# cc-ai/climategan

Measured on AMD Instinct MI355X. Metric: 640x640 images/sec (G+D step): per-domain sample slots per second of the joint Masker+Painter training step (update_G + update_D), global batch 32 per domain, higher is better.
Workload: dtype bf16

## Files before the change

climategan_amd/csrc/conv_gemm.h:

```cpp
#pragma once
#include "cgan_common.h"

struct ConvGemmArgs {
  const uint16_t* x;
  const u32x4* w;
  const float* bias;
  const uint16_t* res;
  const uint16_t* res2;
  uint16_t* y;
  int n, h_in, w_in, cin_s;
  int cout, cout_s, ctiles, ksteps;
  int kh, kw, stride, pad, dil, pad_mode;
  int h_out, w_out, npix;
  int act, has_res, res_ups;
  float slope;
  float* stats;
};

struct ConvGemmCls {
  int koff;
  int kh, kw;
  int offy, offx;
};
struct ConvGemmExtArgs {
  ConvGemmArgs a;
  int cls_s;
  int ksplit;
  int ks_per;
  float* ws;
  int pair;
  ConvGemmCls cls[4];
};
bool conv_gemm_ext_shape_ok(const ConvGemmArgs& a);
int conv_gemm_splitk_plan(const ConvGemmArgs& a);
size_t conv_gemm_splitk_workspace_bytes(const ConvGemmArgs& a, int ksplit);
int conv_gemm_splitk_launch(const ConvGemmArgs& a, int ksplit, float* ws, int dtype, hipStream_t s);
int conv_gemm_cls_launch(const ConvGemmArgs& a, int cls_s, const ConvGemmCls* cls, int dtype, hipStream_t s);
int conv_gemm_pair_launch(const ConvGemmArgs& a, int dtype, hipStream_t s);

bool conv_gemm_applicable(const CganConvDesc* d);
int conv_gemm_launch(const ConvGemmArgs& a, int dtype, hipStream_t s);
bool conv_gemm_res2_ok(const ConvGemmArgs& a, int dtype);
int conv_gemm_stats_chunk_pixels(const ConvGemmArgs& a, int dtype);
bool conv_gemm_big_ok(const ConvGemmArgs& a);
bool conv1x1_allc_ok(const ConvGemmArgs& a);
int conv1x1_allc_launch(const ConvGemmArgs& a, int dtype, hipStream_t s);
int conv_gemm_big_launch(const ConvGemmArgs& a, int dtype, hipStream_t s);
bool conv_gemm_big_pair_ok(const ConvGemmArgs& a, int dtype);
int conv_gemm_big_pair_launch(const ConvGemmArgs& a, int dtype, hipStream_t s);
bool conv1x1_xres_ok(const ConvGemmArgs& a);
int conv1x1_xres_launch(const ConvGemmArgs& a, int dtype, hipStream_t s);

#ifdef __HIPCC__
typedef float f32x2 __attribute__((ext_vector_type(2)));

__device__ __forceinline__ float row16_sum(float v) {
  v += __builtin_bit_cast(float, __builtin_amdgcn_update_dpp(0, __builtin_bit_cast(int, v), 0x128, 0xf, 0xf, false));
  v += __builtin_bit_cast(float, __builtin_amdgcn_update_dpp(0, __builtin_bit_cast(int, v), 0x124, 0xf, 0xf, false));
  v += __builtin_bit_cast(float, __builtin_amdgcn_update_dpp(0, __builtin_bit_cast(int, v), 0x122, 0xf, 0xf, false));
  v += __builtin_bit_cast(float, __builtin_amdgcn_update_dpp(0, __builtin_bit_cast(int, v), 0x121, 0xf, 0xf, false));
  return v;
}

template <typename T, int WC, int WP>
__device__ __forceinline__ void conv_gemm_stats_epilogue(f32x4 (&acc)[WC][WP], const ConvGemmArgs& p, int cout_base,
                                                         int chunk, int j, int g) {
  if (p.bias) {
#pragma unroll
    for (int c = 0; c < WC; ++c) {
      const int chb = cout_base + c * 16 + 4 * g;
      const f32x4 b = chb < p.cout_s ? *reinterpret_cast<const f32x4*>(p.bias + chb) : (f32x4){0.f, 0.f, 0.f, 0.f};
#pragma unroll
      for (int t = 0; t < WP; ++t) acc[c][t] += b;
    }
  }
  constexpr float inv_cnt = 1.f / (float)(WP * 16);
#pragma unroll
  for (int c = 0; c < WC; ++c) {
    f32x2 vr[WP][2];
#pragma unroll
    for (int t = 0; t < WP; ++t) {
#pragma unroll
      for (int hh = 0; hh < 2; ++hh) {
        float r0, r1;
        unpack2<T>(pack2<T>(acc[c][t][2 * hh], acc[c][t][2 * hh + 1]), r0, r1);
        vr[t][hh] = (f32x2){r0, r1};
      }
    }
    f32x2 s0[2] = {vr[0][0], vr[0][1]};
#pragma unroll
    for (int t = 1; t < WP; ++t) {
      s0[0] += vr[t][0];
      s0[1] += vr[t][1];
    }
    float sm[4], sq[4];
#pragma unroll
    for (int r = 0; r < 4; ++r) sm[r] = row16_sum(s0[r >> 1][r & 1]) * inv_cnt;
    const f32x2 m2[2] = {(f32x2){sm[0], sm[1]}, (f32x2){sm[2], sm[3]}};
    f32x2 s1[2];
#pragma unroll
    for (int hh = 0; hh < 2; ++hh) {
      const f32x2 dv = vr[0][hh] - m2[hh];
      s1[hh] = dv * dv;
    }
// ... 141 lines not shown
```

climategan_amd/csrc/conv_gemm.hip:

```cpp
#include "conv_gemm.h"
#include <type_traits>

namespace {

__device__ __attribute__((aligned(16))) unsigned int g_gemm_zeros[4];

constexpr int NSTAGE = 3;
CGAN_KNOB(int, g_gemm_ws, 0);

__device__ __forceinline__ int reflect_i(int i, int n) {
  if (i < 0) i = -i;
  if (i >= n) i = 2 * n - 2 - i;
  return i;
}

template <typename T, int WAVES_C, int WC, int WP, bool REFLECT, int NS = NSTAGE, bool RES2 = false>
__global__ __launch_bounds__(256, 2) void conv_gemm_kernel(ConvGemmArgs p, int npb, int ncb) {
  constexpr int WAVES_P = 4 / WAVES_C;
  constexpr int CT_BLK = WAVES_C * WC;
  constexpr int PT_BLK = WAVES_P * WP;
  constexpr int STAGE_BYTES = (CT_BLK + PT_BLK) * 1024;
  constexpr int W_PER_WAVE = CT_BLK / 4;
  constexpr int P_PER_WAVE = PT_BLK / 4;
  constexpr int DMA_PER_WAVE = W_PER_WAVE + P_PER_WAVE;
  static_assert(CT_BLK % 4 == 0 && PT_BLK % 4 == 0, "tiles must split evenly over the 4 waves");
  extern __shared__ __attribute__((aligned(1024))) unsigned char smem[];

  const int lane = threadIdx.x & 63;
  const int wave = __builtin_amdgcn_readfirstlane(threadIdx.x >> 6);
  const int j = lane & 15;
  const int g = lane >> 4;
  const int wc = wave % WAVES_C, wp = wave / WAVES_C;

  const int xcd = blockIdx.x & 7, slot = blockIdx.x >> 3;
  const int cblk = slot % ncb;
  const int pblk = xcd * ((npb + 7) >> 3) + slot / ncb;
  if (pblk >= npb) return;

  int pbase[P_PER_WAVE], py0[P_PER_WAVE], px0[P_PER_WAVE];
#pragma unroll
  for (int m = 0; m < P_PER_WAVE; ++m) {
    int pix = (pblk * PT_BLK + wave + 4 * m) * 16 + j;
    bool v = pix < p.npix;
    int pc = v ? pix : 0;
    int ox = pc % p.w_out;
    int r = pc / p.w_out;
    int oy = r % p.h_out;
    int nn = r / p.h_out;
    pbase[m] = nn * p.h_in * p.w_in * p.cin_s + g * 8;
    py0[m] = v ? oy * p.stride - p.pad : -(1 << 28);
    px0[m] = ox * p.stride - p.pad;
  }
  const int ccn = p.cin_s >> 5;
  const long zero_off = reinterpret_cast<const unsigned char*>(g_gemm_zeros) - reinterpret_cast<const unsigned char*>(p.x);

  int i_ky = 0, i_kx = 0, i_cc = 0, i_buf = 0;
  auto issue_piece = [&](int piece) {
    unsigned char* buf = smem + i_buf * STAGE_BYTES;
    if (piece < W_PER_WAVE) {
      const int i = wave + 4 * piece;
      const int ct = min(cblk * CT_BLK + i, p.ctiles - 1);
      const u32x4* src = p.w + ((size_t)ct * p.ksteps + (i_ky * p.kw + i_kx) * ccn + i_cc) * 64 + lane;
      __builtin_amdgcn_global_load_lds((const __attribute__((address_space(1))) void*)src,
                                       (__attribute__((address_space(3))) void*)(buf + i * 1024), 16, 0, 0);
    } else {
      const int m = piece - W_PER_WAVE;
      const int i = wave + 4 * m;
      int iy = py0[m] + i_ky * p.dil, ix = px0[m] + i_kx * p.dil;
      bool ok;
      if (REFLECT) {
        ok = py0[m] > -(1 << 27);
        iy = reflect_i(ok ? iy : 0, p.h_in);
        ix = reflect_i(ix, p.w_in);
      } else {
        ok = (unsigned)iy < (unsigned)p.h_in && (unsigned)ix < (unsigned)p.w_in;
      }
      const long off = ok ? (long)(pbase[m] + (iy * p.w_in + ix) * p.cin_s + i_cc * 32) * 2 : zero_off;
      const unsigned char* src = reinterpret_cast<const unsigned char*>(p.x) + off;
      __builtin_amdgcn_global_load_lds((const __attribute__((address_space(1))) void*)src,
                                       (__attribute__((address_space(3))) void*)(buf + (CT_BLK + i) * 1024), 16, 0, 0);
    }
  };
  auto issue_advance = [&]() {
    const int kx1 = i_kx + 1;
    const bool wx = kx1 == p.kw;
    i_kx = wx ? 0 : kx1;
    const int ky1 = i_ky + (wx ? 1 : 0);
    const bool wy = ky1 == p.kh;
    i_ky = wy ? 0 : ky1;
    const int cc1 = i_cc + (wy ? 1 : 0);
    i_cc = cc1 == ccn ? 0 : cc1;
    i_buf = (i_buf + 1 == NS) ? 0 : i_buf + 1;
  };
  auto issue = [&]() {
#pragma unroll
    for (int q = 0; q < DMA_PER_WAVE; ++q) issue_piece(q);
    issue_advance();
  };

  f32x4 acc[WC][WP];
#pragma unroll
  for (int c = 0; c < WC; ++c)
#pragma unroll
    for (int t = 0; t < WP; ++t) acc[c][t] = (f32x4){0.f, 0.f, 0.f, 0.f};

  issue();
  if (NS > 2) issue();
  int r_buf = 0;
  for (int ks = 0; ks < p.ksteps; ++ks) {
    asm volatile("s_waitcnt vmcnt(%0) lgkmcnt(0)" ::"n"((NS - 2) * DMA_PER_WAVE) : "memory");
    __builtin_amdgcn_s_barrier();
    const unsigned char* buf = smem + r_buf * STAGE_BYTES;
    u32x4 a[WC], b[WP];
#pragma unroll
    for (int t = 0; t < WP; ++t)
      b[t] = *reinterpret_cast<const u32x4*>(buf + (CT_BLK + wp * WP + t) * 1024 + lane * 16);
#pragma unroll
    for (int c = 0; c < WC; ++c) a[c] = *reinterpret_cast<const u32x4*>(buf + (wc * WC + c) * 1024 + lane * 16);
    constexpr int NM = WC * WP;
    constexpr int GAP = NM / (DMA_PER_WAVE + 1);
    __builtin_amdgcn_sched_barrier(0);
#pragma unroll
    for (int i = 0; i < NM; ++i) {
      const int c = i / WP, t = i % WP;
      acc[c][t] = mfma16(as_vec8<T>(a[c]), as_vec8<T>(b[t]), acc[c][t]);
      if ((i + 1) % GAP == 0 && (i + 1) / GAP <= DMA_PER_WAVE) {
        issue_piece((i + 1) / GAP - 1);
        __builtin_amdgcn_sched_barrier(0);
      }
    }
    issue_advance();
    r_buf = (r_buf + 1 == NS) ? 0 : r_buf + 1;
  }

  constexpr int ROWB = WC * 64 + 16;
  constexpr int PP = (4 * 4 * 16 * ROWB <= NS * STAGE_BYTES && WP % 4 == 0) ? 4
                     : (4 * 2 * 16 * ROWB <= NS * STAGE_BYTES ? 2 : 1);
  static_assert(4 * PP * 16 * ROWB <= NS * STAGE_BYTES, "epilogue staging does not fit");
  static_assert(WP % PP == 0, "WP must be a multiple of PP");
  asm volatile("s_waitcnt vmcnt(0) lgkmcnt(0)" ::: "memory");
  __builtin_amdgcn_s_barrier();
  unsigned char* stg = smem + wave * (PP * 16 * ROWB);
  const int cout_base = (cblk * CT_BLK + wc * WC) * 16;
  const float* bias_ep = p.bias;
  if (p.stats && (pblk * PT_BLK + wp * WP) * 16 < p.npix) {
    conv_gemm_stats_epilogue<T, WC, WP>(acc, p, cout_base, pblk * WAVES_P + wp, j, g);
    if (p.bias) bias_ep = nullptr;
  }
  conv_gemm_staged_store<T, WC, WP, PP, RES2>(acc, p, stg, (pblk * PT_BLK + wp * WP) * 16, cout_base, bias_ep, lane, j, g);
}

template <typename T, int WC, int WP>
__global__ __launch_bounds__(512, 2) void conv_gemm_k64_kernel(ConvGemmArgs p, int npb, int ncb, int tiles_total) {
  constexpr int CT_BLK = 2 * WC, PT_BLK = 2 * WP;
  constexpr int W_BYTES = CT_BLK * 2048, STAGE_BYTES = (CT_BLK + PT_BLK) * 2048;
  constexpr int NS = 3;
  constexpr int W_PER = CT_BLK / 2, P_PER = PT_BLK / 2, PIECES = W_PER + P_PER;
  static_assert(PIECES <= 63, "vmcnt range");
  extern __shared__ __attribute__((aligned(1024))) unsigned char smem[];

  const int lane = threadIdx.x & 63;
  const int wave = __builtin_amdgcn_readfirstlane(threadIdx.x >> 6);
  const int xcd = blockIdx.x & 7, slot = blockIdx.x >> 3, nslot = gridDim.x >> 3;
  const int per = (tiles_total + 7) >> 3;
  const int t0 = xcd * per;
  const int t1 = min(t0 + per, tiles_total);
  const int my_n = (t1 - t0 > slot) ? (t1 - t0 - slot + nslot - 1) / nslot : 0;
  if (my_n <= 0) return;
  const int first = t0 + slot;
  const int cc2n = p.cin_s >> 6;
  const int n_st = p.kh * p.kw * cc2n;
  const int n_it = my_n * n_st;

  if (wave >= 4) {
    const int pw = wave - 4;
    const int half = pw & 1;
    const int ccn = p.cin_s >> 5;
    const long zero_off = reinterpret_cast<const unsigned char*>(g_gemm_zeros) - reinterpret_cast<const unsigned char*>(p.x);
    const int q = lane >> 3;
    const int kchunk = (lane & 7) ^ (4 * half + ((q >> 1) & 3));
    int poff[P_PER];
    unsigned vmask[P_PER];
    const u32x4* wtile[W_PER];
    auto set_tile = [&](int ti) {
      const int gt = first + ti * nslot;
      const int pblk = gt / ncb;
      const int cblk = gt - pblk * ncb;
#pragma unroll
      for (int m = 0; m < W_PER; ++m)
        wtile[m] = p.w + (size_t)min(cblk * CT_BLK + (pw >> 1) + 2 * m, p.ctiles - 1) * p.ksteps * 64 + half * 64 + lane;
#pragma unroll
      for (int m = 0; m < P_PER; ++m) {
        const int pix = (pblk * PT_BLK + (pw >> 1) + 2 * m) * 16 + 8 * half + q;
        const bool v = pix < p.npix;
        const int pc = v ? pix : 0;
        const int ox = pc % p.w_out;
        const int r = pc / p.w_out;
        const int oy = r % p.h_out;
        const int nn = r / p.h_out;
        const int py0 = oy * p.stride - p.pad, px0 = ox * p.stride - p.pad;
        poff[m] = ((nn * p.h_in * p.w_in + py0 * p.w_in + px0) * p.cin_s + kchunk * 8) * 2;
        unsigned mk = 0;
        for (int ky = 0; ky < p.kh; ++ky)
          for (int kx = 0; kx < p.kw; ++kx) {
            const bool ok = v && (unsigned)(py0 + ky * p.dil) < (unsigned)p.h_in && (unsigned)(px0 + kx * p.dil) < (unsigned)p.w_in;
            mk |= (ok ? 1u : 0u) << (ky * p.kw + kx);
          }
        vmask[m] = mk;
      }
    };
    int i_ky = 0, i_kx = 0, i_cc2 = 0, i_buf = 0, i_st = 0, i_tile = 0, issued = 0;
    auto issue_stage = [&]() {
      unsigned char* buf = smem + i_buf * STAGE_BYTES;
      const int tap = i_ky * p.kw + i_kx;
      const size_t w_ks = (size_t)(tap * ccn + 2 * i_cc2) * 64;
#pragma unroll
      for (int m = 0; m < W_PER; ++m)
        __builtin_amdgcn_global_load_lds((const __attribute__((address_space(1))) void*)(wtile[m] + w_ks),
                                         (__attribute__((address_space(3))) void*)(buf + (pw + 4 * m) * 1024), 16, 0, 0);
      const int tap_off = ((i_ky * p.w_in + i_kx) * p.dil * p.cin_s + i_cc2 * 64) * 2;
#pragma unroll
      for (int m = 0; m < P_PER; ++m) {
        const long off = ((vmask[m] >> tap) & 1u) ? (long)(poff[m] + tap_off) : zero_off;
        const unsigned char* src = reinterpret_cast<const unsigned char*>(p.x) + off;
        __builtin_amdgcn_global_load_lds((const __attribute__((address_space(1))) void*)src,
                                         (__attribute__((address_space(3))) void*)(buf + W_BYTES + (pw + 4 * m) * 1024), 16, 0, 0);
      }
      ++issued;
      i_buf = (i_buf + 1 == NS) ? 0 : i_buf + 1;
      if (++i_st == n_st) {
        i_st = 0; i_ky = 0; i_kx = 0; i_cc2 = 0;
        if (++i_tile < my_n) set_tile(i_tile);
      } else if (++i_kx == p.kw) {
        i_kx = 0;
        if (++i_ky == p.kh) {
          i_ky = 0;
          ++i_cc2;
        }
      }
    };
    set_tile(0);
    for (int s2 = 0; s2 < NS - 1; ++s2)
      if (issued < n_it) issue_stage();
    for (int j = 0; j < n_it; ++j) {
      if (issued - 1 - j >= NS - 2)
        asm volatile("s_waitcnt vmcnt(%0)" ::"n"((NS - 2) * PIECES) : "memory");
      else
        asm volatile("s_waitcnt vmcnt(0)" ::: "memory");
      __builtin_amdgcn_s_barrier();
      if (issued < n_it) issue_stage();
    }
    return;
  }

  const int wc = wave & 1, wp = wave >> 1;
  const int j16 = lane & 15, g = lane >> 4;
  f32x4 acc[WC][WP];
#pragma unroll
  for (int c = 0; c < WC; ++c)
#pragma unroll
    for (int t = 0; t < WP; ++t) acc[c][t] = (f32x4){0.f, 0.f, 0.f, 0.f};
  u32x4 a0[WC], b0[WP], a1[WC], b1[WP];
  int r_buf = 0;
  const int a_off = wc * WC * 2048 + lane * 16;
  int b_off[2];
  {
    const int q = j16 & 7, h = j16 >> 3;
#pragma unroll
    for (int c = 0; c < 2; ++c)
      b_off[c] = W_BYTES + wp * WP * 2048 + 1024 * h + 128 * q + 16 * ((4 * c + g) ^ (4 * h + ((q >> 1) & 3)));
  }
  auto fetch_one = [&](const unsigned char* buf, int c, int qi, u32x4* na, u32x4* nb) {
    if (qi < WP)
      nb[qi] = *reinterpret_cast<const u32x4*>(buf + b_off[c] + qi * 2048);
    else
      na[qi - WP] = *reinterpret_cast<const u32x4*>(buf + a_off + ((qi - WP) * 2 + c) * 1024);
  };
  auto step = [&](const u32x4* ca, const u32x4* cb, u32x4* na, u32x4* nb, int next_half) {
    __builtin_amdgcn_sched_barrier(0);
    if (next_half == 0) {
      asm volatile("s_waitcnt lgkmcnt(0)" ::: "memory");
      __builtin_amdgcn_s_barrier();
      r_buf = (r_buf + 1 == NS) ? 0 : r_buf + 1;
    }
    __builtin_amdgcn_sched_barrier(0);
// ... 34 lines not shown
            int ox = pix % p.w_out;
            int r = pix / p.w_out;
            int oy = r % p.h_out;
            int nn = r / p.h_out;
            rbase = (((size_t)nn * (p.h_out >> 1) + (oy >> 1)) * (p.w_out >> 1) + (ox >> 1)) * p.cout_s;
          } else {
            rbase = (size_t)pix * p.cout_s;
          }
        }
#pragma unroll
        for (int c = 0; c < WC; ++c) {
          const int ch = (cblk * CT_BLK + wc * WC + c) * 16 + 4 * g;
          rv[t][c] = make_uint2(0u, 0u);
          if (pix < p.npix && ch < p.cout_s) rv[t][c] = *reinterpret_cast<const uint2*>(p.res + rbase + ch);
        }
      }
      __builtin_amdgcn_sched_barrier(0);
      __builtin_amdgcn_s_waitcnt(0x0F70);
    }
#pragma unroll
    for (int t = 0; t < WP; ++t) {
      const int pix = (pblk * PT_BLK + wp * WP + t) * 16 + j16;
#pragma unroll
      for (int c = 0; c < WC; ++c) {
        const int ch = (cblk * CT_BLK + wc * WC + c) * 16 + 4 * g;
        float v[4] = {acc[c][t][0], acc[c][t][1], acc[c][t][2], acc[c][t][3]};
        acc[c][t] = (f32x4){0.f, 0.f, 0.f, 0.f};
        if (pix >= p.npix || ch >= p.cout_s) continue;
        if (p.bias) {
#pragma unroll
          for (int r = 0; r < 4; ++r) v[r] += p.bias[ch + r];
        }
        if (p.has_res) {
          float r0, r1;
          unpack2<T>(rv[t][c].x, r0, r1);
          v[0] = cgan_res_apply(v[0], r0, p.has_res); v[1] = cgan_res_apply(v[1], r1, p.has_res);
          unpack2<T>(rv[t][c].y, r0, r1);
          v[2] = cgan_res_apply(v[2], r0, p.has_res); v[3] = cgan_res_apply(v[3], r1, p.has_res);
        }
#pragma unroll
        for (int r = 0; r < 4; ++r) {
          v[r] = act_apply(v[r], p.act, p.slope);
          if (ch + r >= p.cout) v[r] = 0.f;
        }
        u32x2 o;
        o.x = pack2<T>(v[0], v[1]);
        o.y = pack2<T>(v[2], v[3]);
        CGAN_ST_STREAM(o, reinterpret_cast<u32x2*>(p.y + (size_t)pix * p.cout_s + ch));
      }
    }
  };

  for (int ti = 0; ti < my_n; ++ti) {
    first_read(ti > 0);
    for (int st = 0; st + 1 < n_st; ++st) {
      step(a0, b0, a1, b1, 1);
      step(a1, b1, a0, b0, 0);
    }
    step(a0, b0, a1, b1, 1);
    step(a1, b1, a0, b0, -1);
    epilogue(ti);
  }
}

template <typename T, int WC, int WP>
int launch_k64(const ConvGemmArgs& a, hipStream_t s) {
  constexpr int CT_BLK = 2 * WC, PT_BLK = 2 * WP;
  constexpr size_t smem = (size_t)3 * (CT_BLK + PT_BLK) * 2048;
  static bool attr_set = false;
  if (!attr_set) {
    hipError_t e = hipFuncSetAttribute(reinterpret_cast<const void*>(&conv_gemm_k64_kernel<T, WC, WP>),
                                       hipFuncAttributeMaxDynamicSharedMemorySize, 160 * 1024);
    if (e != hipSuccess) {
      cgan_set_error("conv_gemm_k64: hipFuncSetAttribute failed: %s", hipGetErrorString(e));
      return CGAN_ERR_HIP;
    }
    attr_set = true;
  }
  const int npb = ceil_div(ceil_div(a.npix, 16), PT_BLK);
  const int ncb = ceil_div(a.ctiles, CT_BLK);
  const int tiles = npb * ncb;
  const int per = ceil_div(tiles, 8);
  const int nslot = per < 32 ? per : 32;
  hipLaunchKernelGGL((conv_gemm_k64_kernel<T, WC, WP>), dim3(8 * nslot), dim3(512), smem, s, a, npb, ncb, tiles);
  return CGAN_OK;
}
bool k64_ok(const ConvGemmArgs& a) {
  return (a.cin_s & 63) == 0 && a.pad_mode != CGAN_PAD_REFLECT && a.kh * a.kw <= 32 &&
         (long)a.n * a.h_in * a.w_in * a.cin_s < (1L << 30) - (1L << 20);
}


template <typename T, int WAVES_C, int WC, int WP, bool REFLECT, int NS = NSTAGE, bool RES2 = false>
int launch_cfg2(const ConvGemmArgs& a, hipStream_t s) {
  constexpr int WAVES_P = 4 / WAVES_C;
  constexpr int CT_BLK = WAVES_C * WC, PT_BLK = WAVES_P * WP;
  constexpr size_t smem = (size_t)NS * (CT_BLK + PT_BLK) * 1024;
  static bool attr_set = false;
  if (!attr_set) {
    hipError_t e = hipFuncSetAttribute(reinterpret_cast<const void*>(&conv_gemm_kernel<T, WAVES_C, WC, WP, REFLECT, NS, RES2>),
                                       hipFuncAttributeMaxDynamicSharedMemorySize, 160 * 1024);
    if (e != hipSuccess) {
      cgan_set_error("conv_gemm: hipFuncSetAttribute failed: %s", hipGetErrorString(e));
      return CGAN_ERR_HIP;
    }
    attr_set = true;
  }
  const int npb = ceil_div(ceil_div(a.npix, 16), PT_BLK);
  const int ncb = ceil_div(a.ctiles, CT_BLK);
  const int grid = ceil_div(npb, 8) * 8 * ncb;
  hipLaunchKernelGGL((conv_gemm_kernel<T, WAVES_C, WC, WP, REFLECT, NS, RES2>), dim3(grid), dim3(256), smem, s, a, npb, ncb);
  return CGAN_OK;
}

template <typename T, int WAVES_C, int WC, int WP, int NS = NSTAGE>
int launch_cfg(const ConvGemmArgs& a, hipStream_t s) {
  return a.pad_mode == CGAN_PAD_REFLECT ? launch_cfg2<T, WAVES_C, WC, WP, true, NS>(a, s)
                                        : launch_cfg2<T, WAVES_C, WC, WP, false, NS>(a, s);
}

CGAN_KNOB(int, g_gemm_cfg, 0);

enum { KIND_PLAIN = 0, KIND_K64_256x128, KIND_K64_128x256, KIND_BIG, KIND_DIRECT, KIND_XRES };
struct Choice {
  int kind;
  int cfg;
};

Choice choose(const ConvGemmArgs& a, bool bf16) {
  const int ptiles = ceil_div(a.npix, 16);
  const bool no_big = g_gemm_ws == 9;
  const bool no_xres = g_gemm_ws == 9 || g_gemm_ws == 12;
  const int ws = (no_big || no_xres || g_gemm_ws == 13 || g_gemm_ws == 14) ? 0 : g_gemm_ws;
  switch (ws) {
    case 5: if (k64_ok(a)) return {KIND_K64_256x128, 0}; break;
    case 6: if (k64_ok(a)) return {KIND_K64_128x256, 0}; break;
    case 8: if (conv_gemm_big_ok(a)) return {KIND_BIG, 0}; break;
    case 10: if (conv1x1_allc_ok(a)) return {KIND_DIRECT, 0}; break;
    case 11: if (conv1x1_xres_ok(a)) return {KIND_XRES, 0}; break;
    default: break;
  }
  const bool automatic = ws == 0 && g_gemm_cfg == 0;
  (void)bf16;
  if (automatic && !no_big && conv1x1_allc_ok(a) && a.ctiles <= 4 && a.npix >= 16384) return {KIND_DIRECT, 0};
  if (automatic && !no_xres && conv1x1_xres_ok(a) && a.ctiles >= 16 && a.npix >= 16384) return {KIND_XRES, 0};
  const bool long_1x1 = a.kh * a.kw == 1 && g_gemm_ws != 13 &&
                        (g_gemm_ws == 14 ? (a.cin_s >= 2048 || (a.cin_s >= 512 && a.ctiles >= 128))
                                         : (a.cin_s >= 1024 || (a.cin_s >= 512 && a.ctiles >= 128)));
  if (automatic && !no_big && conv_gemm_big_ok(a) && a.npix >= 16384 &&
      ((a.cin_s * a.kh * a.kw >= 4096 && a.cin_s >= 512 && !(a.kh * a.kw >= 9 && a.cin_s >= 2048)) || long_1x1))
    return {KIND_BIG, 0};
  if (automatic && k64_ok(a) && a.kh * a.kw >= 9 && a.cin_s >= 512 && a.npix >= 16384) return {KIND_K64_256x128, 0};
  switch (g_gemm_cfg) {
    case 1: return {KIND_PLAIN, 1};
    case 2: if (a.ctiles <= 16) return {KIND_PLAIN, 2}; break;
    case 3: return {KIND_PLAIN, 3};
    case 4: return {KIND_PLAIN, 4};
    case 5: return {KIND_PLAIN, 5};
    default: break;
  }
  if (a.ctiles <= 4) return {KIND_PLAIN, 1};
  if (a.kh * a.kw == 1 && a.ksteps <= 16) return {KIND_PLAIN, 5};
  if (a.ctiles > 8 && a.ctiles <= 16 && ceil_div(ptiles, 8) >= 384) return {KIND_PLAIN, 2};
  if ((long)ceil_div(ptiles, 16) * ceil_div(a.ctiles, 8) >= 384) return {KIND_PLAIN, 3};
  return {KIND_PLAIN, 4};
}

template <typename T>
int launch(const ConvGemmArgs& a, hipStream_t s) {
  const Choice ch = choose(a, std::is_same<T, BF16>::value);
  switch (ch.kind) {
    case KIND_K64_256x128: return launch_k64<T, 8, 4>(a, s);
    case KIND_K64_128x256: return launch_k64<T, 4, 8>(a, s);
    case KIND_BIG: return conv_gemm_big_launch(a, T::id, s);
    case KIND_DIRECT: return conv1x1_allc_launch(a, T::id, s);
    case KIND_XRES: return conv1x1_xres_launch(a, T::id, s);
    default: break;
  }
  switch (ch.cfg) {
    case 1: return launch_cfg<T, 1, 4, 4>(a, s);
    case 2: return launch_cfg<T, 2, 8, 4>(a, s);
    case 3: return launch_cfg<T, 2, 4, 8>(a, s);
    case 5:
      if (a.has_res == 3) return launch_cfg2<T, 2, 4, 4, false, 2, true>(a, s);
      return launch_cfg<T, 2, 4, 4, 2>(a, s);
    default: return launch_cfg<T, 2, 4, 4>(a, s);
  }
}

}

bool conv_gemm_applicable(const CganConvDesc* d) {
  const int cin_s = cgan_cs(d->c_in), cout_s = cgan_cs(d->c_out);
  const long npix = (long)d->n * d->h_out * d->w_out;
  const long in_elems = (long)d->n * d->h_in * d->w_in * cin_s;
  return (cin_s % 32) == 0 && cout_s >= 64 && !d->in_upsample && npix >= 2048 && in_elems < (1L << 31) - (1L << 20) &&
         (long)ceil_div((int)ceil_div((int)npix, 16), 8) * ceil_div(ceil_div(cout_s, 16), 8) >= 128;
}

CGAN_DEV_ONLY(extern "C" void cgan_debug_set_gemm_cfg(int v) { g_gemm_cfg = v; })
CGAN_DEV_ONLY(extern "C" void cgan_debug_set_gemm_ws(int v) { g_gemm_ws = v; })

int conv_gemm_launch(const ConvGemmArgs& a, int dtype, hipStream_t s) {
  return dtype == CGAN_F16 ? launch<F16>(a, s) : launch<BF16>(a, s);
}

bool conv_gemm_res2_ok(const ConvGemmArgs& a, int dtype) {
  const Choice ch = choose(a, dtype == CGAN_BF16);
  return (ch.kind == KIND_PLAIN && ch.cfg == 5 && a.pad_mode != CGAN_PAD_REFLECT) || ch.kind == KIND_BIG;
}

int conv_gemm_stats_chunk_pixels(const ConvGemmArgs& a, int dtype) {
  const Choice ch = choose(a, dtype == CGAN_BF16);
  if (ch.kind == KIND_XRES) return a.npix % 128 == 0 ? 128 : 0;
  if (ch.kind == KIND_BIG) return a.npix % 64 == 0 ? 64 : 0;
  if (ch.kind != KIND_PLAIN) return 0;
  const int ppb = ch.cfg == 3 ? 128 : 64;
  return a.npix % ppb == 0 ? ppb : 0;
}
```

climategan_amd/csrc/conv_gemm_big.hip:

```cpp
#include "conv_gemm.h"
#include <type_traits>

namespace {

__device__ __attribute__((aligned(16))) unsigned int g_big_zeros[4];

template <typename T, int NW, bool PAIR = false, bool RES2 = false>
__global__ __launch_bounds__(NW * 64, NW / 4) void conv_gemm_big_kernel(ConvGemmArgs p, int npb, int ncb) {
  constexpr int WC = NW == 16 ? 4 : 8;
  constexpr int WP = NW == 4 ? 8 : 4;
  constexpr bool DOUBLE = NW == 4;
  constexpr int CT_BLK = 16, PT_BLK = 16;
  constexpr int STAGE = 32 * 1024;
  constexpr int NSW = 2, NSX = 3;
  constexpr int X_BASE = NSW * STAGE;
  constexpr int NPC = 32 / NW;
  constexpr int NM = WC * WP, NR = WC + WP;
  static_assert(NSW * STAGE + NSX * STAGE == 160 * 1024, "the rings take all of the CU's LDS");
  extern __shared__ __attribute__((aligned(1024))) unsigned char smem[];

  const int lane = threadIdx.x & 63;
  const int wave = __builtin_amdgcn_readfirstlane(threadIdx.x >> 6);
  const int xcd = blockIdx.x & 7, slot = blockIdx.x >> 3;
  const int cblk = slot % ncb;
  const int pblk = xcd * ((npb + 7) >> 3) + slot / ncb;
  if (pblk >= npb) return;

  const int half = wave & 1;
  const int ccn = p.cin_s >> 5;
  const int cc2n = p.cin_s >> 6;
  const int n_st = p.kh * p.kw * cc2n;
  const long zero_off = reinterpret_cast<const unsigned char*>(g_big_zeros) - reinterpret_cast<const unsigned char*>(p.x);
  const u32x4* wsrc[NPC];
  int poff[NPC];
  unsigned vmask[NPC];
  const int csb = PAIR ? p.cin_s / Split<T>::NB : p.cin_s;
  const int xs = PAIR ? Split<T>::NS * csb : p.cin_s;
  const float inv_csb = 1.0f / (float)csb;
  const int kchunk = (lane & 7) ^ (4 * half + (((lane >> 3) >> 1) & 3));
  {
    const int q = lane >> 3;
#pragma unroll
    for (int m = 0; m < NPC; ++m) {
      const int t = (wave >> 1) + (NW / 2) * m;
      wsrc[m] = p.w + (size_t)min(cblk * CT_BLK + t, p.ctiles - 1) * p.ksteps * 64 + half * 64 + lane;
      const int pix = (pblk * PT_BLK + t) * 16 + 8 * half + q;
      const bool v = pix < p.npix;
      const int pc = v ? pix : 0;
      const int ox = pc % p.w_out;
      const int r = pc / p.w_out;
      const int oy = r % p.h_out;
      const int nn = r / p.h_out;
      const int py0 = oy * p.stride - p.pad, px0 = ox * p.stride - p.pad;
      poff[m] = ((nn * p.h_in * p.w_in + py0 * p.w_in + px0) * xs + (PAIR ? 0 : kchunk * 8)) * 2;
      unsigned mk = 0;
      for (int ky = 0; ky < p.kh; ++ky)
        for (int kx = 0; kx < p.kw; ++kx) {
          const bool ok = v && (unsigned)(py0 + ky * p.dil) < (unsigned)p.h_in && (unsigned)(px0 + kx * p.dil) < (unsigned)p.w_in;
          mk |= (ok ? 1u : 0u) << (ky * p.kw + kx);
        }
      vmask[m] = mk;
    }
  }
  struct Cursor {
    int ky, kx, cc2, slot;
  };
  Cursor cx = {0, 0, 0, 0}, cw = {0, 0, 0, 0};
  auto advance = [&](Cursor& c, int nslots) {
    if (++c.kx == p.kw) {
      c.kx = 0;
      if (++c.ky == p.kh) {
        c.ky = 0;
        ++c.cc2;
      }
    }
    c.slot = (c.slot + 1 == nslots) ? 0 : c.slot + 1;
  };
  auto issue_w_piece = [&](int m) {
    const size_t w_ks = (size_t)((cw.ky * p.kw + cw.kx) * ccn + 2 * cw.cc2) * 64;
    __builtin_amdgcn_global_load_lds((const __attribute__((address_space(1))) void*)(wsrc[m] + w_ks),
                                     (__attribute__((address_space(3))) void*)(smem + cw.slot * STAGE + (wave + NW * m) * 1024),
                                     16, 0, 0);
  };
  auto issue_x_piece = [&](int m) {
    const int tap = cx.ky * p.kw + cx.kx;
    int coff = cx.cc2 * 64;
    if (PAIR) {
      const int c = cx.cc2 * 64 + kchunk * 8;
      const int b = (int)(((float)c + 0.5f) * inv_csb);
      coff = Split<T>::xcomp(b) * csb + (c - b * csb);
    }
    const int tap_off = ((cx.ky * p.w_in + cx.kx) * p.dil * xs + coff) * 2;
    const long off = ((vmask[m] >> tap) & 1u) ? (long)(poff[m] + tap_off) : zero_off;
    const unsigned char* src = reinterpret_cast<const unsigned char*>(p.x) + off;
    __builtin_amdgcn_global_load_lds((const __attribute__((address_space(1))) void*)src,
                                     (__attribute__((address_space(3))) void*)(smem + X_BASE + cx.slot * STAGE + (wave + NW * m) * 1024),
                                     16, 0, 0);
  };
  auto issue_w_stage = [&]() {
#pragma unroll
    for (int m = 0; m < NPC; ++m) issue_w_piece(m);
    advance(cw, NSW);
  };
  auto issue_x_stage = [&]() {
#pragma unroll
    for (int m = 0; m < NPC; ++m) issue_x_piece(m);
    advance(cx, NSX);
  };

  constexpr int NWC = CT_BLK / WC;
  const int wc = wave % NWC, wp = wave / NWC;
  const int j16 = lane & 15, g = lane >> 4;
  f32x4 acc[WC][WP];
#pragma unroll
  for (int c = 0; c < WC; ++c)
#pragma unroll
    for (int t = 0; t < WP; ++t) acc[c][t] = (f32x4){0.f, 0.f, 0.f, 0.f};
  const int a_off = wc * WC * 2048 + lane * 16;
  int b_off[2];
  {
    const int q = j16 & 7, h = j16 >> 3;
#pragma unroll
// ... 148 lines not shown
      const f32x4 v0 = *reinterpret_cast<const f32x4*>(stg + pl * ROWB + qc * 32);
      const f32x4 v1 = *reinterpret_cast<const f32x4*>(stg + pl * ROWB + qc * 32 + 16);
      float v[8] = {v0[0], v0[1], v0[2], v0[3], v1[0], v1[1], v1[2], v1[3]};
      if (bias_ep) {
#pragma unroll
        for (int r = 0; r < 4; ++r) {
          v[r] += bb0[r];
          v[4 + r] += bb1[r];
        }
      }
      if (p.has_res) {
        float rsum[8] = {0.f, 0.f, 0.f, 0.f, 0.f, 0.f, 0.f, 0.f};
#pragma unroll
        for (int k = NCC - 1; k >= 0; --k) {
#pragma unroll
          for (int e = 0; e < 4; ++e) {
            float r0, r1;
            unpack2<T>(rs[it][k][e], r0, r1);
            rsum[2 * e] += r0;
            rsum[2 * e + 1] += r1;
          }
        }
#pragma unroll
        for (int r = 0; r < 8; ++r) v[r] += rsum[r];
      }
      act_apply_n(v, p.act, p.slope);
      if (p.cout < p.cout_s) {
#pragma unroll
        for (int r = 0; r < 8; ++r)
          if (ch + r >= p.cout) v[r] = 0.f;
      }
      uint16_t* yp = p.y + (size_t)pix * p.cout_s * NSB + ch;
#pragma unroll
      for (int k = 0; k < NCC; ++k) {
        u32x4 comp;
#pragma unroll
        for (int e = 0; e < 4; ++e) {
          comp[e] = pack2<T>(v[2 * e], v[2 * e + 1]);
          float q0, q1;
          unpack2<T>(comp[e], q0, q1);
          v[2 * e] -= q0;
          v[2 * e + 1] -= q1;
        }
        if (pix < p.npix && ch_ok) *reinterpret_cast<u32x4*>(yp + k * p.cout_s) = comp;
      }
    }
    asm volatile("s_waitcnt lgkmcnt(0)" ::: "memory");
  };
  static_assert(WP / PP == 2, "two staging passes");
  epilogue_pass(std::integral_constant<int, 0>{});
  epilogue_pass(std::integral_constant<int, 1>{});
}

template <typename T, int NW, bool PAIR = false, bool RES2 = false>
int launch_big(const ConvGemmArgs& a, hipStream_t s) {
  constexpr size_t smem = 160 * 1024;
  static bool attr_set = false;
  if (!attr_set) {
    hipError_t e = hipFuncSetAttribute(reinterpret_cast<const void*>(&conv_gemm_big_kernel<T, NW, PAIR, RES2>),
                                       hipFuncAttributeMaxDynamicSharedMemorySize, 160 * 1024);
    if (e != hipSuccess) {
      cgan_set_error("conv_gemm_big: hipFuncSetAttribute failed: %s", hipGetErrorString(e));
      return CGAN_ERR_HIP;
    }
    attr_set = true;
  }
  const int npb = ceil_div(ceil_div(a.npix, 16), 16);
  const int ncb = ceil_div(a.ctiles, 16);
  const int grid = ceil_div(npb, 8) * 8 * ncb;
  hipLaunchKernelGGL((conv_gemm_big_kernel<T, NW, PAIR, RES2>), dim3(grid), dim3(NW * 64), smem, s, a, npb, ncb);
  return CGAN_OK;
}

}

bool conv_gemm_big_ok(const ConvGemmArgs& a) {
  return (a.cin_s & 63) == 0 && a.pad_mode != CGAN_PAD_REFLECT && a.kh * a.kw <= 32 && a.ctiles >= 12 &&
         (long)a.n * a.h_in * a.w_in * a.cin_s < (1L << 30) - (1L << 20);
}

CGAN_KNOB(int, g_big_waves, 8);
CGAN_DEV_ONLY(extern "C" void cgan_debug_set_big_waves(int v) { g_big_waves = v; })

int conv_gemm_big_launch(const ConvGemmArgs& a, int dtype, hipStream_t s) {
  if (g_big_waves == 16 && a.has_res != 3)
    return dtype == CGAN_F16 ? launch_big<F16, 16>(a, s) : launch_big<BF16, 16>(a, s);
  if (a.has_res == 3)
    return dtype == CGAN_F16 ? launch_big<F16, 8, false, true>(a, s) : launch_big<BF16, 8, false, true>(a, s);
  return dtype == CGAN_F16 ? launch_big<F16, 8>(a, s) : launch_big<BF16, 8>(a, s);
}

bool conv_gemm_big_pair_ok(const ConvGemmArgs& a, int dtype) {
  const int nb = cgan_split_blocks(dtype), ns = cgan_split_store_blocks(dtype);
  return (a.cin_s & 63) == 0 && (a.cin_s % nb) == 0 && a.pad_mode != CGAN_PAD_REFLECT && a.kh * a.kw <= 32 && a.ctiles >= 12 &&
         a.npix >= 16384 && a.stats == nullptr &&
         (long)a.n * a.h_in * a.w_in * (a.cin_s / nb) * ns < (1L << 30) - (1L << 20) &&
         (long)a.npix * a.cout_s * ns < (1L << 31);
}
int conv_gemm_big_pair_launch(const ConvGemmArgs& a, int dtype, hipStream_t s) {
  return dtype == CGAN_F16 ? launch_big<F16, 8, true>(a, s) : launch_big<BF16, 8, true>(a, s);
}
```

Before: 58.41.

## Skip dead padding taps per tile in implicit-GEMM conv kernels

For zero-padded same-size stride-1 convolutions, each tile now works out which kernel taps read only padding (rows above or below the image) and builds a compact table of the live taps. The K-loop then iterates only over those taps, which cuts MMA and DMA stages for border tiles in the plain, k64 and big kernels. It also widens the big-kernel selection to cover wide 3x3 convs. The cost is extra per-tile tap computation and new template variants. The persistent k64 kernel also gets uneven per-tile step counts, which adds correctness risk in its producer/consumer schedule.

```diff
diff --git a/climategan_amd/csrc/conv_gemm.h b/climategan_amd/csrc/conv_gemm.h
--- a/climategan_amd/csrc/conv_gemm.h
+++ b/climategan_amd/csrc/conv_gemm.h
@@ -46,10 +46,69 @@
 bool conv1x1_allc_ok(const ConvGemmArgs& a);
 int conv1x1_allc_launch(const ConvGemmArgs& a, int dtype, hipStream_t s);
 int conv_gemm_big_launch(const ConvGemmArgs& a, int dtype, hipStream_t s);
+bool conv_gemm_big_skips(const ConvGemmArgs& a);
 bool conv_gemm_big_pair_ok(const ConvGemmArgs& a, int dtype);
 int conv_gemm_big_pair_launch(const ConvGemmArgs& a, int dtype, hipStream_t s);
 bool conv1x1_xres_ok(const ConvGemmArgs& a);
 int conv1x1_xres_launch(const ConvGemmArgs& a, int dtype, hipStream_t s);
+
+#ifdef __HIPCC__
+#define CGAN_HD __host__ __device__ __forceinline__
+#else
+#define CGAN_HD static inline
+#endif
+struct ConvPadGeom {
+  int h_out, w_out, h_in, w_in, stride, pad, dil, kh, kw;
+};
+CGAN_HD bool conv_pad_tap_dead(int r0, int r1, bool one_row, int c0, int c1, const ConvPadGeom& g, int ky, int kx) {
+  const int ty = ky * g.dil - g.pad, tx = kx * g.dil - g.pad;
+  const bool dead_y = r1 * g.stride + ty < 0 || r0 * g.stride + ty >= g.h_in;
+  const bool dead_x = one_row && (c1 * g.stride + tx < 0 || c0 * g.stride + tx >= g.w_in);
+  return dead_y || dead_x;
+}
+CGAN_HD unsigned conv_pad_dead_taps_rows(int r0, int r1, bool one_row, int c0, int c1, const ConvPadGeom& g) {
+  unsigned m = 0;
+  for (int ky = 0; ky < g.kh; ++ky)
+    for (int kx = 0; kx < g.kw; ++kx)
+      if (conv_pad_tap_dead(r0, r1, one_row, c0, c1, g, ky, kx)) m |= 1u << (ky * g.kw + kx);
+  return m;
+}
+CGAN_HD unsigned conv_pad_dead_taps(int p0, int p1, int npix, const ConvPadGeom& g, bool zero_pad) {
+  const int taps = g.kh * g.kw;
+  if (!zero_pad || taps > 32 || p0 > p1 || p0 < 0) return 0u;
+  if (p0 >= npix) return taps == 32 ? 0xffffffffu : (1u << taps) - 1u;
+  if (p1 >= npix) p1 = npix - 1;
+  const int hw = g.h_out * g.w_out;
+  const int n0 = p0 / hw;
+  if (p1 / hw != n0) return 0u;
+  const int q0 = p0 - n0 * hw, q1 = p1 - n0 * hw;
+  const int r0 = q0 / g.w_out, r1 = q1 / g.w_out;
+  return conv_pad_dead_taps_rows(r0, r1, r0 == r1, q0 - r0 * g.w_out, q1 - r1 * g.w_out, g);
+}
+CGAN_HD int conv_live_tap_table(unsigned dead, int kh, int kw, unsigned long long& table) {
+  table = 0ull;
+  int n = 0;
+  for (int ky = 0; ky < kh; ++ky)
+    for (int kx = 0; kx < kw; ++kx)
+      if (!((dead >> (ky * kw + kx)) & 1u)) {
+        table |= (unsigned long long)((ky << 2) | kx) << (4 * n);
+        ++n;
+      }
+  return n;
+}
+inline ConvPadGeom conv_pad_geom(const ConvGemmArgs& a) {
+  return ConvPadGeom{a.h_out, a.w_out, a.h_in, a.w_in, a.stride, a.pad, a.dil, a.kh, a.kw};
+}
+bool conv_skip_pad_stages_enabled();
+inline bool conv_gemm_pad_skip_applies(const ConvGemmArgs& a, int tile_pixels) {
+  if (!conv_skip_pad_stages_enabled()) return false;
+  if (a.pad_mode != CGAN_PAD_ZERO || a.stride != 1 || a.kh * a.kw == 1 || a.kh > 3 || a.kw > 3 || !(a.kh & 1) || !(a.kw & 1) ||
+      2 * a.pad != a.dil * (a.kh - 1) || 2 * a.pad != a.dil * (a.kw - 1) || a.h_in != a.h_out || a.w_in != a.w_out)
+    return false;
+  if (conv_pad_dead_taps(0, tile_pixels - 1, a.npix, conv_pad_geom(a), true) == 0u) return false;
+  const long dead_pixels = 2L * ((long)a.pad * a.w_out / tile_pixels) * tile_pixels;
+  return dead_pixels * 100 >= 7L * a.kh * a.h_out * a.w_out;
+}
 
 #ifdef __HIPCC__
 typedef float f32x2 __attribute__((ext_vector_type(2)));
diff --git a/climategan_amd/csrc/conv_gemm.hip b/climategan_amd/csrc/conv_gemm.hip
--- a/climategan_amd/csrc/conv_gemm.hip
+++ b/climategan_amd/csrc/conv_gemm.hip
@@ -7,6 +7,8 @@
 
 constexpr int NSTAGE = 3;
 CGAN_KNOB(int, g_gemm_ws, 0);
+CGAN_KNOB(int, g_skip_pad_stages, 1);
+CGAN_DEV_ONLY(int g_last_launch = -1; long g_skip_launches = 0;)
 
 __device__ __forceinline__ int reflect_i(int i, int n) {
   if (i < 0) i = -i;
@@ -14,7 +16,7 @@
   return i;
 }
 
-template <typename T, int WAVES_C, int WC, int WP, bool REFLECT, int NS = NSTAGE, bool RES2 = false>
+template <typename T, int WAVES_C, int WC, int WP, bool REFLECT, int NS = NSTAGE, bool RES2 = false, bool SKIP = false>
 __global__ __launch_bounds__(256, 2) void conv_gemm_kernel(ConvGemmArgs p, int npb, int ncb) {
   constexpr int WAVES_P = 4 / WAVES_C;
   constexpr int CT_BLK = WAVES_C * WC;
@@ -55,6 +57,16 @@
   const long zero_off = reinterpret_cast<const unsigned char*>(g_gemm_zeros) - reinterpret_cast<const unsigned char*>(p.x);
 
   int i_ky = 0, i_kx = 0, i_cc = 0, i_buf = 0;
+  unsigned long long taptbl = 0ull;
+  int nt = 0, i_t = 0, nks = p.ksteps;
+  if constexpr (SKIP) {
+    const ConvPadGeom geo = {p.h_out, p.w_out, p.h_in, p.w_in, p.stride, p.pad, p.dil, p.kh, p.kw};
+    const int p0 = pblk * PT_BLK * 16;
+    nt = conv_live_tap_table(conv_pad_dead_taps(p0, p0 + PT_BLK * 16 - 1, p.npix, geo, !REFLECT), p.kh, p.kw, taptbl);
+    nks = nt * ccn;
+    i_ky = (int)(taptbl & 15u) >> 2;
+    i_kx = (int)(taptbl & 3u);
+  }
   auto issue_piece = [&](int piece) {
     unsigned char* buf = smem + i_buf * STAGE_BYTES;
     if (piece < W_PER_WAVE) {
@@ -82,6 +94,18 @@
     }
   };
   auto issue_advance = [&]() {
+    if constexpr (SKIP) {
+      const int t1 = i_t + 1;
+      const bool wt = t1 == nt;
+      i_t = wt ? 0 : t1;
+      const int cc1 = i_cc + (wt ? 1 : 0);
+      i_cc = cc1 == ccn ? 0 : cc1;
+      const unsigned code = (unsigned)(taptbl >> (4 * i_t)) & 15u;
+      i_ky = (int)(code >> 2);
+      i_kx = (int)(code & 3u);
+      i_buf = (i_buf + 1 == NS) ? 0 : i_buf + 1;
+      return;
+    }
     const int kx1 = i_kx + 1;
     const bool wx = kx1 == p.kw;
     i_kx = wx ? 0 : kx1;
@@ -107,7 +131,7 @@
   issue();
   if (NS > 2) issue();
   int r_buf = 0;
-  for (int ks = 0; ks < p.ksteps; ++ks) {
+  for (int ks = 0; ks < nks; ++ks) {
     asm volatile("s_waitcnt vmcnt(%0) lgkmcnt(0)" ::"n"((NS - 2) * DMA_PER_WAVE) : "memory");
     __builtin_amdgcn_s_barrier();
     const unsigned char* buf = smem + r_buf * STAGE_BYTES;
@@ -150,7 +174,7 @@
   conv_gemm_staged_store<T, WC, WP, PP, RES2>(acc, p, stg, (pblk * PT_BLK + wp * WP) * 16, cout_base, bias_ep, lane, j, g);
 }
 
-template <typename T, int WC, int WP>
+template <typename T, int WC, int WP, bool SKIP = false>
 __global__ __launch_bounds__(512, 2) void conv_gemm_k64_kernel(ConvGemmArgs p, int npb, int ncb, int tiles_total) {
   constexpr int CT_BLK = 2 * WC, PT_BLK = 2 * WP;
   constexpr int W_BYTES = CT_BLK * 2048, STAGE_BYTES = (CT_BLK + PT_BLK) * 2048;
@@ -170,7 +194,11 @@
   const int first = t0 + slot;
   const int cc2n = p.cin_s >> 6;
   const int n_st = p.kh * p.kw * cc2n;
-  const int n_it = my_n * n_st;
+  auto tile_taps = [&](int ti, unsigned long long& tbl) -> int {
+    const ConvPadGeom geo = {p.h_out, p.w_out, p.h_in, p.w_in, p.stride, p.pad, p.dil, p.kh, p.kw};
+    const int p0 = ((first + ti * nslot) / ncb) * (PT_BLK * 16);
+    return conv_live_tap_table(conv_pad_dead_taps(p0, p0 + PT_BLK * 16 - 1, p.npix, geo, true), p.kh, p.kw, tbl);
+  };
 
   if (wave >= 4) {
     const int pw = wave - 4;
@@ -182,7 +210,21 @@
     int poff[P_PER];
     unsigned vmask[P_PER];
     const u32x4* wtile[W_PER];
+    int n_it = my_n * n_st;
+    unsigned long long taptbl = 0ull;
+    int nt = p.kh * p.kw, n_st_t = n_st, i_t = 0;
+    if constexpr (SKIP) {
+      n_it = 0;
+      for (int ti = 0; ti < my_n; ++ti) {
+        unsigned long long tb;
+        n_it += tile_taps(ti, tb) * cc2n;
+      }
+    }
     auto set_tile = [&](int ti) {
+      if constexpr (SKIP) {
+        nt = tile_taps(ti, taptbl);
+        n_st_t = nt * cc2n;
+      }
       const int gt = first + ti * nslot;
       const int pblk = gt / ncb;
       const int cblk = gt - pblk * ncb;
@@ -212,6 +254,11 @@
     int i_ky = 0, i_kx = 0, i_cc2 = 0, i_buf = 0, i_st = 0, i_tile = 0, issued = 0;
     auto issue_stage = [&]() {
       unsigned char* buf = smem + i_buf * STAGE_BYTES;
+      if constexpr (SKIP) {
+        const unsigned code = (unsigned)(taptbl >> (4 * i_t)) & 15u;
+        i_ky = (int)(code >> 2);
+        i_kx = (int)(code & 3u);
+      }
       const int tap = i_ky * p.kw + i_kx;
       const size_t w_ks = (size_t)(tap * ccn + 2 * i_cc2) * 64;
 #pragma unroll
@@ -228,9 +275,14 @@
       }
       ++issued;
       i_buf = (i_buf + 1 == NS) ? 0 : i_buf + 1;
-      if (++i_st == n_st) {
-        i_st = 0; i_ky = 0; i_kx = 0; i_cc2 = 0;
+      if (++i_st == n_st_t) {
+        i_st = 0; i_ky = 0; i_kx = 0; i_cc2 = 0; i_t = 0;
         if (++i_tile < my_n) set_tile(i_tile);
+      } else if (SKIP) {
+        if (++i_t == nt) {
+          i_t = 0;
+          ++i_cc2;
+        }
       } else if (++i_kx == p.kw) {
         i_kx = 0;
         if (++i_ky == p.kh) {
@@ -371,8 +423,13 @@
   };
 
   for (int ti = 0; ti < my_n; ++ti) {
+    int n_st_t = n_st;
+    if constexpr (SKIP) {
+      unsigned long long tb;
+      n_st_t = tile_taps(ti, tb) * cc2n;
+    }
     first_read(ti > 0);
-    for (int st = 0; st + 1 < n_st; ++st) {
+    for (int st = 0; st + 1 < n_st_t; ++st) {
       step(a0, b0, a1, b1, 1);
       step(a1, b1, a0, b0, 0);
     }
@@ -382,13 +439,13 @@
   }
 }
 
-template <typename T, int WC, int WP>
+template <typename T, int WC, int WP, bool SKIP = false>
 int launch_k64(const ConvGemmArgs& a, hipStream_t s) {
   constexpr int CT_BLK = 2 * WC, PT_BLK = 2 * WP;
   constexpr size_t smem = (size_t)3 * (CT_BLK + PT_BLK) * 2048;
   static bool attr_set = false;
   if (!attr_set) {
-    hipError_t e = hipFuncSetAttribute(reinterpret_cast<const void*>(&conv_gemm_k64_kernel<T, WC, WP>),
+    hipError_t e = hipFuncSetAttribute(reinterpret_cast<const void*>(&conv_gemm_k64_kernel<T, WC, WP, SKIP>),
                                        hipFuncAttributeMaxDynamicSharedMemorySize, 160 * 1024);
     if (e != hipSuccess) {
       cgan_set_error("conv_gemm_k64: hipFuncSetAttribute failed: %s", hipGetErrorString(e));
@@ -401,7 +458,7 @@
   const int tiles = npb * ncb;
   const int per = ceil_div(tiles, 8);
   const int nslot = per < 32 ? per : 32;
-  hipLaunchKernelGGL((conv_gemm_k64_kernel<T, WC, WP>), dim3(8 * nslot), dim3(512), smem, s, a, npb, ncb, tiles);
+  hipLaunchKernelGGL((conv_gemm_k64_kernel<T, WC, WP, SKIP>), dim3(8 * nslot), dim3(512), smem, s, a, npb, ncb, tiles);
   return CGAN_OK;
 }
 bool k64_ok(const ConvGemmArgs& a) {
@@ -410,14 +467,14 @@
 }
 
 
-template <typename T, int WAVES_C, int WC, int WP, bool REFLECT, int NS = NSTAGE, bool RES2 = false>
+template <typename T, int WAVES_C, int WC, int WP, bool REFLECT, int NS = NSTAGE, bool RES2 = false, bool SKIP = false>
 int launch_cfg2(const ConvGemmArgs& a, hipStream_t s) {
   constexpr int WAVES_P = 4 / WAVES_C;
   constexpr int CT_BLK = WAVES_C * WC, PT_BLK = WAVES_P * WP;
   constexpr size_t smem = (size_t)NS * (CT_BLK + PT_BLK) * 1024;
   static bool attr_set = false;
   if (!attr_set) {
-    hipError_t e = hipFuncSetAttribute(reinterpret_cast<const void*>(&conv_gemm_kernel<T, WAVES_C, WC, WP, REFLECT, NS, RES2>),
+    hipError_t e = hipFuncSetAttribute(reinterpret_cast<const void*>(&conv_gemm_kernel<T, WAVES_C, WC, WP, REFLECT, NS, RES2, SKIP>),
                                        hipFuncAttributeMaxDynamicSharedMemorySize, 160 * 1024);
     if (e != hipSuccess) {
       cgan_set_error("conv_gemm: hipFuncSetAttribute failed: %s", hipGetErrorString(e));
@@ -428,7 +485,7 @@
   const int npb = ceil_div(ceil_div(a.npix, 16), PT_BLK);
   const int ncb = ceil_div(a.ctiles, CT_BLK);
   const int grid = ceil_div(npb, 8) * 8 * ncb;
-  hipLaunchKernelGGL((conv_gemm_kernel<T, WAVES_C, WC, WP, REFLECT, NS, RES2>), dim3(grid), dim3(256), smem, s, a, npb, ncb);
+  hipLaunchKernelGGL((conv_gemm_kernel<T, WAVES_C, WC, WP, REFLECT, NS, RES2, SKIP>), dim3(grid), dim3(256), smem, s, a, npb, ncb);
   return CGAN_OK;
 }
 
@@ -466,8 +523,9 @@
   const bool long_1x1 = a.kh * a.kw == 1 && g_gemm_ws != 13 &&
                         (g_gemm_ws == 14 ? (a.cin_s >= 2048 || (a.cin_s >= 512 && a.ctiles >= 128))
                                          : (a.cin_s >= 1024 || (a.cin_s >= 512 && a.ctiles >= 128)));
+  const bool wide_3x3 = a.kh * a.kw >= 9 && a.cin_s * a.kh * a.kw >= 2048 && a.ctiles >= 64;
   if (automatic && !no_big && conv_gemm_big_ok(a) && a.npix >= 16384 &&
-      ((a.cin_s * a.kh * a.kw >= 4096 && a.cin_s >= 512 && !(a.kh * a.kw >= 9 && a.cin_s >= 2048)) || long_1x1))
+      ((a.cin_s * a.kh * a.kw >= 4096 && a.cin_s >= 512 && !(a.kh * a.kw >= 9 && a.cin_s >= 2048)) || long_1x1 || wide_3x3))
     return {KIND_BIG, 0};
   if (automatic && k64_ok(a) && a.kh * a.kw >= 9 && a.cin_s >= 512 && a.npix >= 16384) return {KIND_K64_256x128, 0};
   switch (g_gemm_cfg) {
@@ -488,6 +546,14 @@
 template <typename T>
 int launch(const ConvGemmArgs& a, hipStream_t s) {
   const Choice ch = choose(a, std::is_same<T, BF16>::value);
+  const bool skip = (ch.kind == KIND_K64_256x128 && conv_gemm_pad_skip_applies(a, 128)) ||
+                    (ch.kind == KIND_PLAIN && ch.cfg == 3 && conv_gemm_pad_skip_applies(a, 256));
+  CGAN_DEV_ONLY(g_last_launch = ch.kind * 256 + ch.cfg * 16 + ((skip || (ch.kind == KIND_BIG && conv_gemm_big_skips(a))) ? 1 : 0);)
+  if (skip) {
+    CGAN_DEV_ONLY(++g_skip_launches;)
+    if (ch.kind == KIND_K64_256x128) return launch_k64<T, 8, 4, true>(a, s);
+    return launch_cfg2<T, 2, 4, 8, false, NSTAGE, false, true>(a, s);
+  }
   switch (ch.kind) {
     case KIND_K64_256x128: return launch_k64<T, 8, 4>(a, s);
     case KIND_K64_128x256: return launch_k64<T, 4, 8>(a, s);
@@ -519,6 +585,24 @@
 
 CGAN_DEV_ONLY(extern "C" void cgan_debug_set_gemm_cfg(int v) { g_gemm_cfg = v; })
 CGAN_DEV_ONLY(extern "C" void cgan_debug_set_gemm_ws(int v) { g_gemm_ws = v; })
+CGAN_DEV_ONLY(extern "C" void cgan_debug_set_skip_pad_stages(int v) { g_skip_pad_stages = v; })
+bool conv_skip_pad_stages_enabled() { return g_skip_pad_stages != 0; }
+#ifdef CGAN_DEV
+long conv_gemm_big_skip_launches();
+extern "C" int cgan_debug_gemm_last_launch() { return g_last_launch; }
+extern "C" long cgan_debug_skip_pad_launches() { return g_skip_launches + conv_gemm_big_skip_launches(); }
+extern "C" unsigned cgan_debug_pad_dead_taps(int p0, int p1, int npix, int h_out, int w_out, int h_in, int w_in, int stride,
+                                             int pad, int dil, int kh, int kw, int zero_pad) {
+  const ConvPadGeom g = {h_out, w_out, h_in, w_in, stride, pad, dil, kh, kw};
+  return conv_pad_dead_taps(p0, p1, npix, g, zero_pad != 0);
+}
+extern "C" int cgan_debug_live_tap_table(unsigned dead, int kh, int kw, unsigned long long* table) {
+  unsigned long long t = 0ull;
+  const int n = conv_live_tap_table(dead, kh, kw, t);
+  if (table) *table = t;
+  return n;
+}
+#endif
 
 int conv_gemm_launch(const ConvGemmArgs& a, int dtype, hipStream_t s) {
   return dtype == CGAN_F16 ? launch<F16>(a, s) : launch<BF16>(a, s);
diff --git a/climategan_amd/csrc/conv_gemm_big.hip b/climategan_amd/csrc/conv_gemm_big.hip
--- a/climategan_amd/csrc/conv_gemm_big.hip
+++ b/climategan_amd/csrc/conv_gemm_big.hip
@@ -5,7 +5,7 @@
 
 __device__ __attribute__((aligned(16))) unsigned int g_big_zeros[4];
 
-template <typename T, int NW, bool PAIR = false, bool RES2 = false>
+template <typename T, int NW, bool PAIR = false, bool RES2 = false, bool SKIP = false>
 __global__ __launch_bounds__(NW * 64, NW / 4) void conv_gemm_big_kernel(ConvGemmArgs p, int npb, int ncb) {
   constexpr int WC = NW == 16 ? 4 : 8;
   constexpr int WP = NW == 4 ? 8 : 4;
@@ -29,7 +29,14 @@
   const int half = wave & 1;
   const int ccn = p.cin_s >> 5;
   const int cc2n = p.cin_s >> 6;
-  const int n_st = p.kh * p.kw * cc2n;
+  unsigned long long taptbl = 0ull;
+  int nt = p.kh * p.kw;
+  if constexpr (SKIP) {
+    const ConvPadGeom geo = {p.h_out, p.w_out, p.h_in, p.w_in, p.stride, p.pad, p.dil, p.kh, p.kw};
+    const int p0 = pblk * PT_BLK * 16;
+    nt = conv_live_tap_table(conv_pad_dead_taps(p0, p0 + PT_BLK * 16 - 1, p.npix, geo, true), p.kh, p.kw, taptbl);
+  }
+  const int n_st = nt * cc2n;
   const long zero_off = reinterpret_cast<const unsigned char*>(g_big_zeros) - reinterpret_cast<const unsigned char*>(p.x);
   const u32x4* wsrc[NPC];
   int poff[NPC];
@@ -63,11 +70,23 @@
     }
   }
   struct Cursor {
-    int ky, kx, cc2, slot;
-  };
-  Cursor cx = {0, 0, 0, 0}, cw = {0, 0, 0, 0};
+    int ky, kx, cc2, slot, t;
+  };
+  Cursor cx = {0, 0, 0, 0, 0}, cw = {0, 0, 0, 0, 0};
+  if constexpr (SKIP) {
+    cx.ky = cw.ky = (int)(taptbl & 15u) >> 2;
+    cx.kx = cw.kx = (int)(taptbl & 3u);
+  }
   auto advance = [&](Cursor& c, int nslots) {
-    if (++c.kx == p.kw) {
+    if constexpr (SKIP) {
+      if (++c.t == nt) {
+        c.t = 0;
+        ++c.cc2;
+      }
+      const unsigned code = (unsigned)(taptbl >> (4 * c.t)) & 15u;
+      c.ky = (int)(code >> 2);
+      c.kx = (int)(code & 3u);
+    } else if (++c.kx == p.kw) {
       c.kx = 0;
       if (++c.ky == p.kh) {
         c.ky = 0;
@@ -322,12 +341,12 @@
   epilogue_pass(std::integral_constant<int, 1>{});
 }
 
-template <typename T, int NW, bool PAIR = false, bool RES2 = false>
+template <typename T, int NW, bool PAIR = false, bool RES2 = false, bool SKIP = false>
 int launch_big(const ConvGemmArgs& a, hipStream_t s) {
   constexpr size_t smem = 160 * 1024;
   static bool attr_set = false;
   if (!attr_set) {
-    hipError_t e = hipFuncSetAttribute(reinterpret_cast<const void*>(&conv_gemm_big_kernel<T, NW, PAIR, RES2>),
+    hipError_t e = hipFuncSetAttribute(reinterpret_cast<const void*>(&conv_gemm_big_kernel<T, NW, PAIR, RES2, SKIP>),
                                        hipFuncAttributeMaxDynamicSharedMemorySize, 160 * 1024);
     if (e != hipSuccess) {
       cgan_set_error("conv_gemm_big: hipFuncSetAttribute failed: %s", hipGetErrorString(e));
@@ -338,7 +357,7 @@
   const int npb = ceil_div(ceil_div(a.npix, 16), 16);
   const int ncb = ceil_div(a.ctiles, 16);
   const int grid = ceil_div(npb, 8) * 8 * ncb;
-  hipLaunchKernelGGL((conv_gemm_big_kernel<T, NW, PAIR, RES2>), dim3(grid), dim3(NW * 64), smem, s, a, npb, ncb);
+  hipLaunchKernelGGL((conv_gemm_big_kernel<T, NW, PAIR, RES2, SKIP>), dim3(grid), dim3(NW * 64), smem, s, a, npb, ncb);
   return CGAN_OK;
 }
 
@@ -352,7 +371,17 @@
 CGAN_KNOB(int, g_big_waves, 8);
 CGAN_DEV_ONLY(extern "C" void cgan_debug_set_big_waves(int v) { g_big_waves = v; })
 
+CGAN_DEV_ONLY(static long g_big_skip_launches = 0; long conv_gemm_big_skip_launches() { return g_big_skip_launches; })
+
+bool conv_gemm_big_skips(const ConvGemmArgs& a) {
+  return !(g_big_waves == 16 && a.has_res != 3) && a.has_res != 3 && conv_gemm_pad_skip_applies(a, 256);
+}
+
 int conv_gemm_big_launch(const ConvGemmArgs& a, int dtype, hipStream_t s) {
+  if (conv_gemm_big_skips(a)) {
+    CGAN_DEV_ONLY(++g_big_skip_launches;)
+    return dtype == CGAN_F16 ? launch_big<F16, 8, false, false, true>(a, s) : launch_big<BF16, 8, false, false, true>(a, s);
+  }
   if (g_big_waves == 16 && a.has_res != 3)
     return dtype == CGAN_F16 ? launch_big<F16, 16>(a, s) : launch_big<BF16, 16>(a, s);
   if (a.has_res == 3)
```

After: 58.16. Within noise of the previous version (-0.4%).
